# excamera/alfalfa

Hardware: AMD Instinct MI355X
Metric: 1080p macroblocks/s decode (bit-exact vs reference) (higher is better)
Workload: dtype u8

## Files before the change

### alfalfa_amd/csrc/kernels.hip

```cpp
#include <hip/hip_runtime.h>
#include <algorithm>
#include <cstddef>

#include <cstdlib>

#include "device_types.h"
#include "vp8_math.hh"
#include "coeff_pack.hh"
#include "recon_inl.hh"

namespace aa {
namespace {
using namespace recon;

constexpr int kLanes = 64;

enum : int { DC_PRED, V_PRED, H_PRED, TM_PRED, B_PRED, NEARESTMV, NEARMV, ZEROMV, NEWMV, SPLITMV };

struct alignas( 16 ) ResidualLds {
  union {
    int16_t cf[25][16];
    int16_t res[24][16];
  };
  int16_t im[24][16];
  uint8_t map[32];
};

__device__ void compute_residual( const aa_mb_info & mb, const aa_dev_frame & f, ResidualLds & L, const int lane )
{
  uint32_t * z = reinterpret_cast<uint32_t *>( &L.cf[0][0] );
  for ( int i = lane; i < 200; i += kLanes ) z[i] = 0;
  const uint32_t mask = mb.nz_mask;
  if ( lane < 25 && ( ( mask >> lane ) & 1u ) ) L.map[lane == 24 ? 0 : __popc( mask & ( ( 1u << lane ) - 1u ) ) + static_cast<int>( mask >> 24 )] = static_cast<uint8_t>( lane );
  __syncthreads();
  const uint16_t * q = f.quant[mb.segment_id & 3];
  if ( f.packed ) {
    const int16_t * const w = f.coeffs + ( static_cast<size_t>( mb.reserved ) << 32 | mb.coeff_index );
    uint16_t * const scr = reinterpret_cast<uint16_t *>( &L.im[0][0] );
    if ( lane < 25 ) scr[lane] = ( ( mask >> lane ) & 1u ) ? static_cast<uint16_t>( w[lane] ) : 0u;
    __syncthreads();
    if ( lane < 25 ) {
      uint32_t off = pack::kMaskSlots;
      if ( lane != 24 ) { off += __popc( scr[24] ); for ( int b = 0; b < lane; b++ ) off += __popc( scr[b] ); }
      scr[32 + lane] = static_cast<uint16_t>( off );
    }
    __syncthreads();
    for ( int k = lane; k < 25 * 16; k += kLanes ) {
      const int blk = k >> 4, e = k & 15;
      const uint32_t m = scr[blk], zz = pack::zigzag_of( e );
      if ( ( m >> zz ) & 1u ) {
        const int base = blk < 16 ? 0 : ( blk < 24 ? 4 : 2 );
        L.cf[blk][e] = static_cast<int16_t>( dequant( w[scr[32 + blk] + __popc( m & ( ( 1u << zz ) - 1u ) )], q[base + ( e ? 1 : 0 )] ) );
      }
    }
  } else {
    const int n = __popc( mask ) * 16;
    const int16_t * src = f.coeffs + static_cast<size_t>( mb.coeff_index ) * 16;
    for ( int k = lane; k < n; k += kLanes ) {
      const int blk = L.map[k >> 4], e = k & 15;
      const int base = blk < 16 ? 0 : ( blk < 24 ? 4 : 2 );
      L.cf[blk][e] = static_cast<int16_t>( dequant( src[k], q[base + ( e ? 1 : 0 )] ) );
    }
  }
  __syncthreads();
  if ( mb.flags & AA_MB_HAS_Y2 ) {
    if ( lane < 4 ) {
      const Quad v = iwht_pass1( L.cf[24][lane], L.cf[24][lane + 4], L.cf[24][lane + 8], L.cf[24][lane + 12] );
      L.im[0][lane] = static_cast<int16_t>( v.v0 ); L.im[0][lane + 4] = static_cast<int16_t>( v.v1 );
      L.im[0][lane + 8] = static_cast<int16_t>( v.v2 ); L.im[0][lane + 12] = static_cast<int16_t>( v.v3 );
    }
    __syncthreads();
    if ( lane < 4 ) {
      const int o = lane * 4;
      const Quad v = iwht_pass2( L.im[0][o], L.im[0][o + 1], L.im[0][o + 2], L.im[0][o + 3] );
      L.cf[o + 0][0] = static_cast<int16_t>( v.v0 ); L.cf[o + 1][0] = static_cast<int16_t>( v.v1 );
      L.cf[o + 2][0] = static_cast<int16_t>( v.v2 ); L.cf[o + 3][0] = static_cast<int16_t>( v.v3 );
    }
    __syncthreads();
  }
  for ( int t = lane; t < 96; t += kLanes ) {
    const int blk = t >> 2, i = t & 3;
    const Quad v = idct_pass1( L.cf[blk][i], L.cf[blk][i + 4], L.cf[blk][i + 8], L.cf[blk][i + 12] );
    L.im[blk][i * 4 + 0] = static_cast<int16_t>( v.v0 ); L.im[blk][i * 4 + 1] = static_cast<int16_t>( v.v1 );
    L.im[blk][i * 4 + 2] = static_cast<int16_t>( v.v2 ); L.im[blk][i * 4 + 3] = static_cast<int16_t>( v.v3 );
  }
  __syncthreads();
  for ( int t = lane; t < 96; t += kLanes ) {
    const int blk = t >> 2, i = t & 3;
    const Quad v = idct_pass2( L.im[blk][i], L.im[blk][i + 4], L.im[blk][i + 8], L.im[blk][i + 12] );
    L.res[blk][i * 4 + 0] = static_cast<int16_t>( v.v0 ); L.res[blk][i * 4 + 1] = static_cast<int16_t>( v.v1 );
    L.res[blk][i * 4 + 2] = static_cast<int16_t>( v.v2 ); L.res[blk][i * 4 + 3] = static_cast<int16_t>( v.v3 );
  }
  __syncthreads();
}

__device__ __forceinline__ int clampi( int v, int lo, int hi ) { return v < lo ? lo : ( v > hi ? hi : v ); }

__device__ __forceinline__ void load_taps( int frac, int ( &t )[6] )
{
  for ( int i = 0; i < 6; i++ ) t[i] = sixtap_coeff( frac, i );
}

__device__ __forceinline__ uint32_t bytes_at( const uint32_t d0, const uint32_t d1, const uint32_t d2, const int s )
{
  const int q = s >> 2, sh = s & 3;
  const uint32_t lo = q == 0 ? d0 : ( q == 1 ? d1 : d2 );
  const uint32_t hi = q == 0 ? d1 : ( q == 1 ? d2 : 0u );
  return __builtin_amdgcn_alignbyte( hi, lo, sh );
}
__device__ __forceinline__ uint32_t sixtap_x4( uint32_t d0, uint32_t d1, uint32_t d2, const int o, const int frac, const uint32_t t0123, const uint32_t t45 )
{
  if ( frac == 0 ) return bytes_at( d0, d1, d2, o + 2 );
  d0 ^= 0x80808080u; d1 ^= 0x80808080u; d2 ^= 0x80808080u;
  uint32_t out = 0;
#pragma unroll
  for ( int k = 0; k < 4; k++ ) {
    const int a = static_cast<int>( bytes_at( d0, d1, d2, o + k ) ), b = static_cast<int>( bytes_at( d0, d1, d2, o + k + 4 ) );
    int v = __builtin_amdgcn_sdot4( a, static_cast<int>( t0123 ), __builtin_amdgcn_sdot4( b, static_cast<int>( t45 ), 16384 + 64, false ), false ) >> 7;
    asm volatile( "" : "+v"( v ) );
    out |= static_cast<uint32_t>( clamp255( v ) ) << ( 8 * k );
  }
  return out;
}

struct alignas( 16 ) InterLds {
  ResidualLds r;
  alignas( 16 ) uint8_t pred[384];
  union {
    struct {
      uint32_t sw[24][9][3];
      uint32_t st[24][4][3];
      int16_t unit[24][6];
    };
    struct {
      uint32_t wy[21][6], wc[2][13][4];
      uint32_t ty[16][6], tc[2][8][4];
    };
  };
};

__device__ __forceinline__ void recon_inter_body( const aa_dev_frame & f, const unsigned bx, const unsigned max_mbs, InterLds & L, const bool split_only )
{
  const unsigned total = static_cast<unsigned>( f.mbw ) * f.mbh;
  const unsigned chunk = ( max_mbs + 7u ) >> 3;
  const unsigned mi = ( bx & 7u ) * chunk + ( bx >> 3 );
  if ( mi >= total ) return;
  const aa_mb_info & mb = f.mbs[mi];
  if ( !( mb.flags & AA_MB_INTER ) ) return;
  if ( split_only && mb.y_mode != SPLITMV ) return;
  const int lane = threadIdx.x;
  const int col = mi % f.mbw, row = mi / f.mbw;
  const int pw = f.mbw * 16, ph = f.mbh * 16, cw = pw >> 1, ch = ph >> 1;
  const bool has_res = mb.flags & AA_MB_HAS_NONZERO;
  const uint8_t * const * ref = f.ref[mb.ref_frame & 3];
  const bool whole = mb.y_mode != SPLITMV;
  const int mvx = mb.u.mv[0][0], mvy = mb.u.mv[0][1];
  const int cmx = chroma_mv( 4 * mvx ), cmy = chroma_mv( 4 * mvy );
// ... 796 lines not shown
      if ( on && !inside ) {
        uint8_t * by = &S.wy[0][0];
        for ( int i = l; i < 21 * 24; i += 16 ) {
          const int r = i / 24, c = i % 24;
          by[i] = ref_y[static_cast<size_t>( clampi( syy + r, 0, ph - 1 ) ) * pw + clampi( sxy + c, 0, pw - 1 )];
        }
        uint8_t * bc = &S.wc[0][0][0];
        for ( int i = l; i < 2 * 13 * 16; i += 16 ) {
          const int pl = i / 208, e = i % 208, r = e >> 4, c = e & 15;
          bc[i] = ( pl ? ref_v : ref_u )[static_cast<size_t>( clampi( syc + r, 0, ch - 1 ) ) * cw + clampi( sxc + c, 0, cw - 1 )];
        }
      }
    }
  }
  const int oy = inside ? ( sxy & 3 ) : 0, oc = inside ? ( sxc & 3 ) : 0;
  __syncthreads();

  const bool luma_general = __any( on && ( ( mvx | mvy ) & 7 ) != 0 ), chroma_general = __any( on && ( ( cmx | cmy ) & 7 ) != 0 );
  const uint8_t * const wyb = &S.wy[0][0]; const uint8_t * const wcb = &S.wc[0][0][0];
  uint8_t * const tyb = &S.ty[0][0]; uint8_t * const tcb = &S.tc[0][0][0];
  if ( on && luma_general ) {
    const int frac = mvx & 7;
    const uint32_t t0 = L.taps[2 * frac], t1 = L.taps[2 * frac + 1];
#pragma unroll
    for ( int k = 0; k < 6; k++ ) {
      const int t = l + 16 * k;
      if ( k == 5 && t >= 84 ) continue;
      const int r = t >> 2, g = t & 3;
      const uint8_t * sp = wyb + r * 24 + g * 4;
      const uint32_t o4 = sixtap_x4_lane( *reinterpret_cast<const uint32_t *>( sp ), *reinterpret_cast<const uint32_t *>( sp + 4 ), *reinterpret_cast<const uint32_t *>( sp + 8 ), oy, frac, t0, t1 );
      uint8_t * tb = tyb + ( g * 4 ) * 24 + r;
      tb[0] = static_cast<uint8_t>( o4 ); tb[24] = static_cast<uint8_t>( o4 >> 8 ); tb[48] = static_cast<uint8_t>( o4 >> 16 ); tb[72] = static_cast<uint8_t>( o4 >> 24 );
    }
  }
  if ( on && chroma_general ) {
    const int frac = cmx & 7;
    const uint32_t t0 = L.taps[2 * frac], t1 = L.taps[2 * frac + 1];
#pragma unroll
    for ( int k = 0; k < 4; k++ ) {
      const int j = l + 16 * k;
      if ( k == 3 && j >= 52 ) continue;
      const int pl = j >= 26 ? 1 : 0, e = j - 26 * pl, r = e >> 1, g = e & 1;
      const uint8_t * sp = wcb + pl * 208 + r * 16 + g * 4;
      const uint32_t o4 = sixtap_x4_lane( *reinterpret_cast<const uint32_t *>( sp ), *reinterpret_cast<const uint32_t *>( sp + 4 ), *reinterpret_cast<const uint32_t *>( sp + 8 ), oc, frac, t0, t1 );
      uint8_t * tb = tcb + pl * 128 + ( g * 4 ) * 16 + r;
      tb[0] = static_cast<uint8_t>( o4 ); tb[16] = static_cast<uint8_t>( o4 >> 8 ); tb[32] = static_cast<uint8_t>( o4 >> 16 ); tb[48] = static_cast<uint8_t>( o4 >> 24 );
    }
  }
  uint4 copy_y = make_uint4( 0, 0, 0, 0 ); uint2 copy_c = make_uint2( 0, 0 );
  if ( !luma_general && on ) {
    const uint2 * rp = reinterpret_cast<const uint2 *>( wyb + ( l + 2 ) * 24 );
    const uint2 a = rp[0], b = rp[1], c = rp[2];
    const bool q = oy + 2 >= 4; const int sft = ( oy + 2 ) & 3;
    const uint32_t e0 = q ? a.y : a.x, e1 = q ? b.x : a.y, e2 = q ? b.y : b.x, e3 = q ? c.x : b.y, e4 = q ? c.y : c.x;
    copy_y = make_uint4( __builtin_amdgcn_alignbyte( e1, e0, sft ), __builtin_amdgcn_alignbyte( e2, e1, sft ),
                         __builtin_amdgcn_alignbyte( e3, e2, sft ), __builtin_amdgcn_alignbyte( e4, e3, sft ) );
  }
  if ( !chroma_general && on ) {
    const int pl = l >> 3, r = l & 7;
    const uint2 * rp = reinterpret_cast<const uint2 *>( wcb + pl * 208 + ( r + 2 ) * 16 );
    const uint2 a = rp[0], b = rp[1];
    const bool q = oc + 2 >= 4; const int sft = ( oc + 2 ) & 3;
    const uint32_t e0 = q ? a.y : a.x, e1 = q ? b.x : a.y, e2 = q ? b.y : b.x;
    copy_c = make_uint2( __builtin_amdgcn_alignbyte( e1, e0, sft ), __builtin_amdgcn_alignbyte( e2, e1, sft ) );
  }
  __syncthreads();
  if ( !luma_general && on ) *reinterpret_cast<uint4 *>( S.pred + l * 16 ) = copy_y;
  if ( !chroma_general && on ) *reinterpret_cast<uint2 *>( S.pred + 256 + ( l >> 3 ) * 64 + ( l & 7 ) * 8 ) = copy_c;
  if ( on && luma_general ) {
    const int frac = mvy & 7;
    const uint32_t t0 = L.taps[2 * frac], t1 = L.taps[2 * frac + 1];
#pragma unroll
    for ( int k = 0; k < 4; k++ ) {
      const int t = l + 16 * k, c = t >> 2, i = t & 3;
      const uint8_t * sp = tyb + c * 24 + i * 4;
      const uint32_t o4 = sixtap_x4_lane( *reinterpret_cast<const uint32_t *>( sp ), *reinterpret_cast<const uint32_t *>( sp + 4 ), *reinterpret_cast<const uint32_t *>( sp + 8 ), 0, frac, t0, t1 );
      uint8_t * pb = S.pred + ( i * 4 ) * 16 + c;
      pb[0] = static_cast<uint8_t>( o4 ); pb[16] = static_cast<uint8_t>( o4 >> 8 ); pb[32] = static_cast<uint8_t>( o4 >> 16 ); pb[48] = static_cast<uint8_t>( o4 >> 24 );
    }
  }
  if ( on && chroma_general ) {
    const int frac = cmy & 7;
    const uint32_t t0 = L.taps[2 * frac], t1 = L.taps[2 * frac + 1];
#pragma unroll
    for ( int k = 0; k < 2; k++ ) {
      const int j = l + 16 * k, pl = j >> 4, c = ( j >> 1 ) & 7, i = j & 1;
      const uint8_t * sp = tcb + pl * 128 + c * 16 + i * 4;
      const uint32_t o4 = sixtap_x4_lane( *reinterpret_cast<const uint32_t *>( sp ), *reinterpret_cast<const uint32_t *>( sp + 4 ), *reinterpret_cast<const uint32_t *>( sp + 8 ), 0, frac, t0, t1 );
      uint8_t * pb = S.pred + 256 + pl * 64 + ( i * 4 ) * 8 + c;
      pb[0] = static_cast<uint8_t>( o4 ); pb[8] = static_cast<uint8_t>( o4 >> 8 ); pb[16] = static_cast<uint8_t>( o4 >> 16 ); pb[24] = static_cast<uint8_t>( o4 >> 24 );
    }
  }
  __syncthreads();

  if ( on ) {
    uint32_t o[4];
#pragma unroll
    for ( int k = 0; k < 4; k++ ) {
      const uint32_t p4 = *reinterpret_cast<const uint32_t *>( S.pred + l * 16 + 4 * k );
      const uint32_t out = has_res ? add_residual_x4( p4, &S.res[( l >> 2 ) * 4 + k][( l & 3 ) * 4] ) : p4;
      o[k] = out;
    }
    *reinterpret_cast<uint4 *>( f.cur[0] + static_cast<size_t>( row * 16 + l ) * pw + col * 16 ) = make_uint4( o[0], o[1], o[2], o[3] );
    const int pl = l >> 3, r = l & 7;
    uint32_t oc2[2];
#pragma unroll
    for ( int k = 0; k < 2; k++ ) {
      const uint32_t p4 = *reinterpret_cast<const uint32_t *>( S.pred + 256 + pl * 64 + r * 8 + 4 * k );
      const uint32_t out = has_res ? add_residual_x4( p4, &S.res[16 + pl * 4 + ( r >> 2 ) * 2 + k][( r & 3 ) * 4] ) : p4;
      oc2[k] = out;
    }
    *reinterpret_cast<uint2 *>( f.cur[1 + pl] + static_cast<size_t>( row * 8 + r ) * cw + col * 8 ) = make_uint2( oc2[0], oc2[1] );
  }
}

__global__ __launch_bounds__( kLanes ) void k_recon_inter4( const aa_frame_list list, const unsigned max_quads )
{
  __builtin_amdgcn_s_setprio( 3 );

  __shared__ Inter4Lds L;
  recon_inter4_body( *list.f[blockIdx.y], blockIdx.x, max_quads, L );
}

constexpr int kStripMbs = 8;
constexpr int kStripRow = 16 + 16 * kStripMbs;
constexpr int kStripRpi = 16 / kStripMbs;
static_assert( ( kStripRow / 16 ) % 2 == 1, "odd multiple of 16: consecutive rows start on different banks" );
struct alignas( 16 ) LfStrip {
  uint8_t c[12][kStripRow];
  uint8_t y[20][kStripRow];
  uint8_t halo_y[16][4];
  uint8_t halo_c[2][8][4];
  uint8_t pad[32];
};
struct alignas( 16 ) LfStripLds { LfStrip slot[4]; };

__device__ __forceinline__ uint64_t load_u64_shared( const uint8_t * p )
{
  return __hip_atomic_load( reinterpret_cast<const uint64_t *>( p ), __ATOMIC_RELAXED, __HIP_MEMORY_SCOPE_AGENT );
}

__device__ __forceinline__ void lf_edges_pk( pk2 ( &v )[20], const LfParamsPk & P, const pk2 g0, const pk2 g1, const pk2 g23 )
{
  if ( __any( g0 != 0u ) ) lf_edge_pk( P, true, g0, v[0], v[1], v[2], v[3], v[4], v[5], v[6], v[7] );
  if ( __any( g1 != 0u ) ) {
    lf_edge_pk( P, false, g1, v[4], v[5], v[6], v[7], v[8], v[9], v[10], v[11] );
    if ( __any( g23 != 0u ) ) {
      lf_edge_pk( P, false, g23, v[8], v[9], v[10], v[11], v[12], v[13], v[14], v[15] );
      lf_edge_pk( P, false, g23, v[12], v[13], v[14], v[15], v[16], v[17], v[18], v[19] );
    }
  }
}

__device__ __forceinline__ void loopfilter_strip_row( const aa_frame_list & list, const int group, const int row, const int mbh_max, const int mbw_max,
                                                       aa_sync_ws * ws, uint8_t * bnd, LfStripLds & S, const int dbg, const int home_xcc )
{
  const int lane = threadIdx.x, slot = lane >> 4, l = lane & 15;
  const aa_dev_frame & f0 = *list.f[group * 4];
  const int mbh = f0.mbh;
  if ( row >= mbh ) return;
  const aa_dev_frame * const fp = list.f[group * 4 + slot];
  const bool frame_on = fp != nullptr && fp->loop_filter_level != 0;
  if ( !__any( frame_on ) ) return;
  const aa_dev_frame & f = fp ? *fp : f0;
  LfStrip & T = S.slot[slot];
  int * const progress = ws->progress + group * mbh_max;
  const int mbw = f0.mbw, pw = mbw * 16, cw = pw >> 1;
  const int y0 = row * 16, cy0 = row * 8;
  const int sharp = f.sharpness; const bool key = f.key_frame;
  const bool last_row = row == mbh - 1;
  const bool luma = l < 8;
  const int k8 = l & 7, cp = k8 >> 2, cj = k8 & 3;
  uint8_t * const vrow = luma ? &T.y[4 + 2 * l][16] : &T.c[4 + 2 * cj][16 + 8 * kStripMbs * cp];
  uint8_t * const vhalo = luma ? &T.halo_y[2 * l][0] : &T.halo_c[cp][2 * cj][0];
  uint8_t * const hcol = luma ? &T.y[0][16 + 2 * l] : &T.c[0][16 + 8 * kStripMbs * cp + 2 * cj];
  const int mbstep = luma ? 16 : 8;
  const int brow = l / kStripMbs, bchunk = l % kStripMbs;
  uint8_t * const gy = f.cur[0] + static_cast<size_t>( y0 + brow ) * pw + 16 * bchunk;
  uint8_t * const gu = f.cur[1] + static_cast<size_t>( cy0 + brow ) * cw + 8 * bchunk;
  uint8_t * const gv = f.cur[2] + static_cast<size_t>( cy0 + brow ) * cw + 8 * bchunk;
  uint8_t * const sy = &T.y[4 + brow][16 + 16 * bchunk];
  uint8_t * const sc = &T.c[4 + brow][16 + 8 * bchunk];
  const int bl = l & 7, bq = ( bl - 4 ) & 3;
  uint8_t * const bsrc = bl < 4 ? &T.y[16 + bl][16] : &T.c[8 + 2 * ( bq & 1 )][16 + 8 * kStripMbs * ( bq >> 1 )];
  uint8_t * const btop = bl < 4 ? &T.y[bl][16] : &T.c[2 * ( bq & 1 )][16 + 8 * kStripMbs * ( bq >> 1 )];
  const int bstep = bl < 4 ? 16 : 8;
  const size_t bnd_row = ( static_cast<size_t>( group * 4 + slot ) * mbh_max + row ) * mbw_max;
  uint8_t * const bnd_own = bnd + bnd_row * 128 + 16 * bl;
  const uint8_t * const bnd_top = bnd + ( bnd_row - mbw_max ) * 128 + 16 * bl;
  const int fq = l >> 2, fr = l & 3;
  const int fix_off = fq == 0 ? 16 * fr + 12 : 64 + 32 * ( fq - 1 ) + 8 * fr + 4;
  uint8_t * const fix_src0 = fq == 0 ? &T.halo_y[12 + fr][0] : &T.halo_c[( fq - 1 ) & 1][4 + fr][0];
  uint8_t * const fix_srck = fq == 0 ? &T.y[16 + fr][16 - 4] : &T.c[8 + fr][16 + 8 * kStripMbs * ( ( fq - 1 ) & 1 ) - 4];
  const int fix_step = fq == 0 ? 16 : 8;
  uint8_t * const fy = f.cur[0] + static_cast<size_t>( y0 + l ) * pw - 4;
  uint8_t * const fc = f.cur[1 + ( l >> 3 )] + static_cast<size_t>( cy0 + ( l & 7 ) ) * cw - 4;
  const aa_mb_info * const mbrow = f.mbs + static_cast<size_t>( row ) * mbw;

  const int n_strips = ( mbw + kStripMbs - 1 ) / kStripMbs;
  uint4 py[kStripMbs]; uint2 pc[kStripMbs];
#pragma unroll
  for ( int i = 0; i < kStripMbs; i++ ) { py[i] = make_uint4( 0, 0, 0, 0 ); pc[i] = make_uint2( 0, 0 ); }
  auto prefetch = [&]( const int s ) {
    const bool in = frame_on && !( dbg & 2 ) && s * kStripMbs + bchunk < mbw;
    if ( in ) {
#pragma unroll
      for ( int i = 0; i < kStripMbs; i++ ) py[i] = *reinterpret_cast<const uint4 *>( gy + static_cast<size_t>( kStripRpi * i ) * pw + 16 * kStripMbs * s );
#pragma unroll
      for ( int i = 0; i < kStripMbs / 2; i++ ) pc[i] = *reinterpret_cast<const uint2 *>( gu + static_cast<size_t>( kStripRpi * i ) * cw + 8 * kStripMbs * s );
#pragma unroll
      for ( int i = 0; i < kStripMbs / 2; i++ ) pc[kStripMbs / 2 + i] = *reinterpret_cast<const uint2 *>( gv + static_cast<size_t>( kStripRpi * i ) * cw + 8 * kStripMbs * s );
    }
  };
  prefetch( 0 );
  int info = frame_on ? *reinterpret_cast<const uint16_t *>( &mbrow[0].flags ) : 0;
  int seen = row > 0 ? 0 : mbw;
  LfParamsPk P = lf_params_pk( lf_params( 1, sharp, key ) );
  int p_level = -1;
  for ( int s = 0; s < n_strips; s++ ) {
    const int nmb = min( kStripMbs, mbw - s * kStripMbs );
    if ( s > 0 ) {
      *reinterpret_cast<uint32_t *>( &T.halo_y[l][0] ) = *reinterpret_cast<const uint32_t *>( &T.y[4 + l][16 + 16 * kStripMbs - 4] );
      *reinterpret_cast<uint32_t *>( &T.halo_c[l >> 3][l & 7][0] ) = *reinterpret_cast<const uint32_t *>( &T.c[4 + ( l & 7 )][16 + 8 * kStripMbs * ( l >> 3 ) + 8 * kStripMbs - 4] );
      __syncthreads();
    }
#pragma unroll
    for ( int i = 0; i < kStripMbs; i++ ) *reinterpret_cast<uint4 *>( sy + kStripRpi * kStripRow * i ) = py[i];
#pragma unroll
    for ( int i = 0; i < kStripMbs / 2; i++ ) { *reinterpret_cast<uint2 *>( sc + kStripRpi * kStripRow * i ) = pc[i]; *reinterpret_cast<uint2 *>( sc + kStripRpi * kStripRow * i + 8 * kStripMbs ) = pc[kStripMbs / 2 + i]; }
    __syncthreads();

    for ( int k = 0; k < nmb; k++ ) {
      const int col = s * kStripMbs + k;
      const int level = info >> 8;
      const bool active = level != 0;
      const bool inner = !( info & AA_MB_LF_SKIP_INNER );
      const bool more = col + 1 < mbw;
      const int info_next = ( frame_on && more ) ? *reinterpret_cast<const uint16_t *>( &mbrow[col + 1].flags ) : 0;
      const int need = col + 1;
      if ( row > 0 && seen < need ) seen = poll_progress( &progress[row - 1] );
      const bool any_active = __any( active );
      if ( !__all( level == p_level ) ) { P = lf_params_pk( lf_params( active ? level : 1, sharp, key ) ); p_level = level; }
      const pk2 g_on = active ? ~0u : 0u, g_in = ( active && inner ) ? ~0u : 0u, g_in23 = ( active && inner && luma ) ? ~0u : 0u;

      if ( any_active && !( dbg & 4 ) ) {
        uint8_t * const ra = vrow + mbstep * k;
        uint8_t * const ha = k == 0 ? vhalo : ra - 4;
        uint8_t * const hb = k == 0 ? vhalo + 4 : ra + kStripRow - 4;
        uint32_t a[5], b[5];
        a[0] = *reinterpret_cast<const uint32_t *>( ha ); b[0] = *reinterpret_cast<const uint32_t *>( hb );
        { const uint2 u = *reinterpret_cast<const uint2 *>( ra ); a[1] = u.x; a[2] = u.y; }
        { const uint2 u = *reinterpret_cast<const uint2 *>( ra + 8 ); a[3] = u.x; a[4] = u.y; }
        { const uint2 u = *reinterpret_cast<const uint2 *>( ra + kStripRow ); b[1] = u.x; b[2] = u.y; }
        { const uint2 u = *reinterpret_cast<const uint2 *>( ra + kStripRow + 8 ); b[3] = u.x; b[4] = u.y; }
        pk2 v[20];
#pragma unroll
        for ( int d = 0; d < 5; d++ ) {
          v[4 * d] = pk_from_bytes<0>( a[d], b[d] ); v[4 * d + 1] = pk_from_bytes<1>( a[d], b[d] );
          v[4 * d + 2] = pk_from_bytes<2>( a[d], b[d] ); v[4 * d + 3] = pk_from_bytes<3>( a[d], b[d] );
        }
        lf_edges_pk( v, P, col > 0 ? g_on : 0u, g_in, g_in23 );
#pragma unroll
        for ( int d = 0; d < 5; d++ ) pk_to_dwords( v[4 * d], v[4 * d + 1], v[4 * d + 2], v[4 * d + 3], a[d], b[d] );
        if ( active ) {
          *reinterpret_cast<uint32_t *>( ha ) = a[0]; *reinterpret_cast<uint32_t *>( hb ) = b[0];
          *reinterpret_cast<uint2 *>( ra ) = make_uint2( a[1], a[2] ); *reinterpret_cast<uint2 *>( ra + kStripRow ) = make_uint2( b[1], b[2] );
          if ( luma ) { *reinterpret_cast<uint2 *>( ra + 8 ) = make_uint2( a[3], a[4] ); *reinterpret_cast<uint2 *>( ra + kStripRow + 8 ) = make_uint2( b[3], b[4] ); }
        }
      }
      __syncthreads();
      if ( frame_on && !last_row && col > 0 && l < 12 && !( dbg & 1 ) ) {
        const uint8_t * src = k == 0 ? fix_src0 : fix_srck + fix_step * k;
        *reinterpret_cast<uint32_t *>( bnd + ( bnd_row + col - 1 ) * 128 + fix_off ) = *reinterpret_cast<const uint32_t *>( src );
      }

      if ( row > 0 ) {
        if ( !( dbg & 16 ) ) wait_for_row_above( true, need, seen, 2, ws, progress, group, row, mbh, home_xcc, lf_min_polls( dbg ), lf_max_wait_ticks( dbg ) );

        if ( frame_on && l < 8 && !( dbg & 8 ) ) {
          const uint8_t * src = bnd_top + static_cast<size_t>( col ) * 128;
          const uint64_t lo = load_u64_shared( src ), hi = load_u64_shared( src + 8 );
          uint8_t * dst = btop + bstep * k;
          if ( bl < 4 ) { *reinterpret_cast<uint64_t *>( dst ) = lo; *reinterpret_cast<uint64_t *>( dst + 8 ) = hi; }
          else { *reinterpret_cast<uint64_t *>( dst ) = lo; *reinterpret_cast<uint64_t *>( dst + kStripRow ) = hi; }
        }
      }
      publish_progress( lane == 0 && col > 0 && !lf_fault_injected( dbg, row ), &progress[row], col );
      if ( k == 0 && s + 1 < n_strips ) prefetch( s + 1 );
      __syncthreads();

      if ( any_active && !( dbg & 4 ) ) {
        uint8_t * const hc = hcol + mbstep * k;
        pk2 v[20];
#pragma unroll
        for ( int r = 0; r < 20; r++ ) v[r] = pk_from_u16( *reinterpret_cast<const uint16_t *>( hc + kStripRow * r ) );
        lf_edges_pk( v, P, row > 0 ? g_on : 0u, g_in, g_in23 );
        if ( active ) {
#pragma unroll
          for ( int r = 1; r < 12; r++ ) *reinterpret_cast<uint16_t *>( hc + kStripRow * r ) = static_cast<uint16_t>( pk_to_u16( v[r] ) );
          if ( luma ) {
#pragma unroll
            for ( int r = 12; r < 20; r++ ) *reinterpret_cast<uint16_t *>( hc + kStripRow * r ) = static_cast<uint16_t>( pk_to_u16( v[r] ) );
          }
        }
      }
      __syncthreads();

      if ( frame_on && !( dbg & 1 ) ) {
        if ( !last_row ) {
          if ( l < 8 ) {
            const uint8_t * src = bsrc + bstep * k;
            uint4 q;
            if ( bl < 4 ) q = *reinterpret_cast<const uint4 *>( src );
            else { const uint2 u0 = *reinterpret_cast<const uint2 *>( src ), u1 = *reinterpret_cast<const uint2 *>( src + kStripRow ); q = make_uint4( u0.x, u0.y, u1.x, u1.y ); }
            *reinterpret_cast<uint4 *>( bnd_own + static_cast<size_t>( col ) * 128 ) = q;
          }
        }
        if ( k == 0 && s > 0 ) {
          if ( l < 12 || last_row ) *reinterpret_cast<uint32_t *>( fy + 16 * kStripMbs * s ) = *reinterpret_cast<const uint32_t *>( &T.halo_y[l][0] );
          if ( ( l & 7 ) < 4 || last_row ) *reinterpret_cast<uint32_t *>( fc + 8 * kStripMbs * s ) = *reinterpret_cast<const uint32_t *>( &T.halo_c[l >> 3][l & 7][0] );
        }
        if ( k == nmb - 1 && bchunk < nmb ) {
#pragma unroll
          for ( int i = 0; i < 20 / kStripRpi; i++ ) {
            if ( ( ( i + 1 ) * kStripRpi > 4 || row > 0 ) && ( i * kStripRpi < 16 || last_row ) )
              *reinterpret_cast<uint4 *>( gy + ( static_cast<ptrdiff_t>( kStripRpi * i ) - 4 ) * pw + 16 * kStripMbs * s ) = *reinterpret_cast<const uint4 *>( sy + kStripRpi * kStripRow * i - 4 * kStripRow );
          }
#pragma unroll
          for ( int i = 0; i < 12 / kStripRpi; i++ ) {
            if ( ( ( i + 1 ) * kStripRpi > 4 || row > 0 ) && ( i * kStripRpi < 8 || last_row ) ) {
              *reinterpret_cast<uint2 *>( gu + ( static_cast<ptrdiff_t>( kStripRpi * i ) - 4 ) * cw + 8 * kStripMbs * s ) = *reinterpret_cast<const uint2 *>( sc + kStripRpi * kStripRow * i - 4 * kStripRow );
              *reinterpret_cast<uint2 *>( gv + ( static_cast<ptrdiff_t>( kStripRpi * i ) - 4 ) * cw + 8 * kStripMbs * s ) = *reinterpret_cast<const uint2 *>( sc + kStripRpi * kStripRow * i - 4 * kStripRow + 8 * kStripMbs );
            }
          }
        }
      }
      info = info_next;
      __syncthreads();
    }
  }
  publish_progress( lane == 0 && !lf_fault_injected( dbg, row ), &progress[row], mbw );
}

__device__ __forceinline__ void loopfilter_rows4_body( const aa_frame_list & list, const int n_groups, const int mbh_max, const int mbw_max, aa_sync_ws * ws, uint8_t * bnd,
                                                        const int n_xcd, LfStripLds & S, int & s_ticket, const int dbg )
{
  const int xcc = xcc_id();
  if ( xcc >= n_xcd ) { if ( threadIdx.x == 0 ) atomicExch( &ws->error, 3 ); return; }
  for ( ;; ) {
    const int t = take_ticket( ws, xcc, &s_ticket, threadIdx.x );
    const int mine = xcc < n_groups ? ( n_groups - xcc + n_xcd - 1 ) / n_xcd : 0;
    if ( t >= mine * mbh_max ) return;
    loopfilter_strip_row( list, ( t % mine ) * n_xcd + xcc, t / mine, mbh_max, mbw_max, ws, bnd, S, dbg, xcc );
  }
}

__global__ __launch_bounds__( kLanes ) __attribute__( ( amdgpu_waves_per_eu( 2 ) ) ) void k_loopfilter_rows4( const aa_frame_list list, const int n_groups, const int mbh_max, const int mbw_max, aa_sync_ws * ws, uint8_t * bnd,
                                                                 const int n_xcd, const int dbg )
{
  __builtin_amdgcn_s_setprio( 3 );

  __shared__ LfStripLds S;
  __shared__ int s_ticket;
  loopfilter_rows4_body( list, n_groups, mbh_max, mbw_max, ws, bnd, n_xcd, S, s_ticket, dbg );
}

__global__ void k_probe_xcds( int * out )
{
  if ( threadIdx.x == 0 ) atomicAdd( &out[xcc_id() & 15], 1 );
}

__global__ void k_probe_concurrency( uint32_t * counter, uint32_t * seen, uint32_t n, unsigned long long timeout, int slot )
{
  if ( threadIdx.x || blockIdx.x ) return;
  __hip_atomic_fetch_add( counter, 1u, __ATOMIC_RELAXED, __HIP_MEMORY_SCOPE_AGENT );
  const unsigned long long t0 = wall_clock64();
  uint32_t m;
  while ( ( m = __hip_atomic_load( counter, __ATOMIC_RELAXED, __HIP_MEMORY_SCOPE_AGENT ) ) < n && wall_clock64() - t0 < timeout ) __builtin_amdgcn_s_sleep( 32 );
  seen[slot] = m;
}

__global__ void k_check_tickets( aa_sync_ws * ws, const int n_groups, const int mbh_max, const int n_xcd )
{
  if ( threadIdx.x != 0 || blockIdx.x != 0 ) return;
  for ( int x = 0; x < n_xcd; x++ ) {
    const int mine = x < n_groups ? ( n_groups - x + n_xcd - 1 ) / n_xcd : 0;
    const int t = __hip_atomic_load( &ws->ticket[x], __ATOMIC_RELAXED, __HIP_MEMORY_SCOPE_AGENT );
    if ( t < mine * mbh_max && atomicCAS( &ws->error, 0, 5 ) == 0 ) { ws->where[0] = x; ws->where[1] = t; ws->where[2] = mine * mbh_max; }
  }
}

__global__ void k_bind_rasters( const aa_raster_binding * b, int n )
{
  const int i = blockIdx.x * blockDim.x + threadIdx.x;
  if ( i >= n ) return;
  aa_dev_frame * f = b[i].job;
  for ( int p = 0; p < 3; p++ ) f->cur[p] = b[i].cur[p];
  for ( int r = 1; r < 4; r++ ) for ( int p = 0; p < 3; p++ ) f->ref[r][p] = b[i].ref[r - 1][p];
}

__global__ __launch_bounds__( 256 ) void k_gather_rasters( const aa_gather_job * jobs, uint8_t * staging, size_t stride )
{
  const aa_gather_job J = jobs[blockIdx.y];
  const uint4 * src = reinterpret_cast<const uint4 *>( J.src );
  uint4 * dst = reinterpret_cast<uint4 *>( staging + stride * blockIdx.y );
  const size_t n16 = J.bytes >> 4;
  for ( size_t i = size_t( blockIdx.x ) * 256 + threadIdx.x; i < n16; i += size_t( gridDim.x ) * 256 ) dst[i] = src[i];
  if ( blockIdx.x == 0 && threadIdx.x < ( J.bytes & 15 ) ) staging[stride * blockIdx.y + ( n16 << 4 ) + threadIdx.x] = J.src[( n16 << 4 ) + threadIdx.x];
}

constexpr int kRgbCy = 76309, kRgbCrv = 104574, kRgbCgu = 25642, kRgbCgv = 53281, kRgbCbu = 132213;

template <int ESZ, int N>
__device__ inline void rgb_store( uint8_t * p, const uint32_t ( &e )[N], const int n, const bool fast )
{
  static_assert( ( N * ESZ ) % 16 == 0, "whole 16-byte pieces" );
  if ( fast ) {
    uint32_t w[N * ESZ / 4];
#pragma unroll
    for ( int i = 0; i < N * ESZ / 4; i++ ) {
      if ( ESZ == 1 ) w[i] = e[4 * i] | e[4 * i + 1] << 8 | e[4 * i + 2] << 16 | e[4 * i + 3] << 24;
      else if ( ESZ == 2 ) w[i] = ( e[2 * i] & 0xFFFFu ) | e[2 * i + 1] << 16;
      else w[i] = e[i];
    }
    uint4 * q = reinterpret_cast<uint4 *>( p );
#pragma unroll
    for ( int i = 0; i < N * ESZ / 16; i++ ) q[i] = make_uint4( w[4 * i], w[4 * i + 1], w[4 * i + 2], w[4 * i + 3] );
    return;
  }
#pragma unroll
  for ( int i = 0; i < N; i++ )
    if ( i < n )
#pragma unroll
      for ( int b = 0; b < ESZ; b++ ) p[i * ESZ + b] = static_cast<uint8_t>( e[i] >> ( 8 * b ) );
}

template <int F>
__global__ __launch_bounds__( 256 ) void k_render_rgb( const aa_rgb_job * jobs, const uint32_t * table )
{
  constexpr bool kFloat = F >= AA_RGB_F16_CHW;
  constexpr int kEsz = F == AA_RGB_F32_CHW ? 4 : F >= AA_RGB_F16_CHW ? 2 : 1;
  __shared__ uint32_t T[kFloat ? 768 : 1];
  if ( kFloat ) {
    for ( int i = threadIdx.x; i < 768; i += 256 ) T[i] = table[i];
    __syncthreads();
  }
  const aa_rgb_job & J = jobs[blockIdx.y];
  const uint32_t groups = J.groups, w = J.width, h = J.height;
  const uint32_t t = blockIdx.x * 256u + threadIdx.x;
  if ( t >= groups * ( ( h + 1 ) >> 1 ) ) return;
  const int k = static_cast<int>( t / groups ), x0 = static_cast<int>( t - uint32_t( k ) * groups ) * 16;
  const int cw = static_cast<int>( ( w + 1 ) >> 1 ), ch = static_cast<int>( ( h + 1 ) >> 1 );
  const int j0 = x0 >> 1, je = min( j0 + 8, cw - 1 );
  const int crow[3] = { max( k - 1, 0 ), k, min( k + 1, ch - 1 ) };
  int c[2][3][9];
#pragma unroll
  for ( int p = 0; p < 2; p++ )
#pragma unroll
    for ( int r = 0; r < 3; r++ ) {
      const uint8_t * row = J.plane[1 + p] + size_t( crow[r] ) * J.stride_c;
      const uint2 q = *reinterpret_cast<const uint2 *>( row + j0 );
      c[p][r][8] = row[je];
#pragma unroll
      for ( int i = 0; i < 8; i++ ) {
        const int b = static_cast<int>( ( ( i < 4 ? q.x : q.y ) >> ( 8 * ( i & 3 ) ) ) & 255u );
        c[p][r][i] = j0 + i > je ? c[p][r][8] : b;
      }
    }
  const int n = min( 16, static_cast<int>( w ) - x0 );
  for ( int r = 0; r < 2; r++ ) {
    const int y = 2 * k + r;
    if ( y >= static_cast<int>( h ) ) continue;
    const uint4 yq = *reinterpret_cast<const uint4 *>( J.plane[0] + size_t( y ) * J.stride_y + x0 );
    const uint32_t yw[4] = { yq.x, yq.y, yq.z, yq.w };
    int v[2][9];
#pragma unroll
    for ( int p = 0; p < 2; p++ )
#pragma unroll
      for ( int i = 0; i < 9; i++ ) v[p][i] = 3 * c[p][1][i] + c[p][r ? 2 : 0][i];
    uint32_t R[16], G[16], B[16];
#pragma unroll
    for ( int i = 0; i < 16; i++ ) {
      const int Y = static_cast<int>( ( yw[i >> 2] >> ( 8 * ( i & 3 ) ) ) & 255u );
      const int j = i >> 1;
      const int u8 = ( i & 1 ) ? v[0][j] + v[0][j + 1] : 2 * v[0][j];
      const int v8 = ( i & 1 ) ? v[1][j] + v[1][j + 1] : 2 * v[1][j];
      const int yt = 8 * kRgbCy * ( Y - 16 ), ut = u8 - 1024, vt = v8 - 1024;
      R[i] = static_cast<uint32_t>( min( max( ( yt + kRgbCrv * vt + ( 1 << 18 ) ) >> 19, 0 ), 255 ) );
      G[i] = static_cast<uint32_t>( min( max( ( yt - kRgbCgu * ut - kRgbCgv * vt + ( 1 << 18 ) ) >> 19, 0 ), 255 ) );
      B[i] = static_cast<uint32_t>( min( max( ( yt + kRgbCbu * ut + ( 1 << 18 ) ) >> 19, 0 ), 255 ) );
    }
    uint8_t * const row = J.dst + y * J.row_stride;
    if ( F == AA_RGB_U8_HWC3 || F == AA_RGB_U8_HWC4 ) {
      constexpr int C = F == AA_RGB_U8_HWC3 ? 3 : 4;
      uint32_t e[16 * C];
#pragma unroll
      for ( int i = 0; i < 16; i++ ) {
        e[C * i] = R[i]; e[C * i + 1] = G[i]; e[C * i + 2] = B[i];
        if ( C == 4 ) e[C * i + 3] = 255u;
      }
      uint8_t * const p = row + x0 * C;
      rgb_store<1, 16 * C>( p, e, n * C, n == 16 && !( reinterpret_cast<uintptr_t>( p ) & 15 ) );
    } else {
#pragma unroll
      for ( int ci = 0; ci < 3; ci++ ) {
        const uint32_t * const src = ci == 0 ? R : ci == 1 ? G : B;
        uint32_t e[16];
#pragma unroll
        for ( int i = 0; i < 16; i++ ) e[i] = kFloat ? T[ci * 256 + src[i]] : src[i];
        uint8_t * const p = row + ci * J.plane_stride + x0 * kEsz;
        rgb_store<kEsz, 16>( p, e, n, n == 16 && !( reinterpret_cast<uintptr_t>( p ) & 15 ) );
      }
    }
  }
}

}

__global__ __launch_bounds__( 256 ) void k_lf_relevel( const aa_mb_info * src, aa_mb_info * dst, unsigned nmb, uint32_t levels )
{
  const unsigned i = blockIdx.x * blockDim.x + threadIdx.x;
  if ( i >= nmb ) return;
  const uint4 * s = reinterpret_cast<const uint4 *>( src + i );
  uint4 * d = reinterpret_cast<uint4 *>( dst + i );
  uint4 head = s[0];
  const uint32_t seg = ( head.x >> 24 ) & 3u;
  head.y = ( head.y & 0xFFFF00FFu ) | ( ( ( levels >> ( 8 * seg ) ) & 255u ) << 8 );
  d[0] = head;
  for ( int k = 1; k < 5; k++ ) d[k] = s[k];
}
static_assert( sizeof( aa_mb_info ) == 80, "k_lf_relevel copies five 16-byte pieces" );

int launch_lf_relevel( const aa_mb_info * src, aa_mb_info * dst, unsigned nmb, uint32_t levels, void * stream )
{
  hipLaunchKernelGGL( k_lf_relevel, dim3( ( nmb + 255 ) / 256 ), dim3( 256 ), 0, static_cast<hipStream_t>( stream ), src, dst, nmb, levels );
  return static_cast<int>( hipGetLastError() );
}

int launch_gather_rasters( const aa_gather_job * jobs, int n, uint8_t * staging, size_t stride, size_t max_bytes, void * stream )
{
  const unsigned per = static_cast<unsigned>( std::min<size_t>( 64, std::max<size_t>( 1, max_bytes / ( 256 * 16 * 4 ) ) ) );
  for ( int base = 0; base < n; base += 32768 ) {
    const int cnt = std::min( 32768, n - base );
    hipLaunchKernelGGL( k_gather_rasters, dim3( per, cnt ), dim3( 256 ), 0, static_cast<hipStream_t>( stream ), jobs + base, staging + stride * base, stride );
    if ( hipError_t e = hipGetLastError() ) return static_cast<int>( e );
  }
  return 0;
}

int launch_render_rgb( const aa_rgb_job * jobs, int n, int format, const uint32_t * table, uint32_t max_threads, void * stream )
{
  const unsigned blocks = ( max_threads + 255u ) / 256u;
  const hipStream_t st = static_cast<hipStream_t>( stream );
  for ( int base = 0; base < n; base += 32768 ) {
    const dim3 grid( blocks, std::min( 32768, n - base ) );
    switch ( format ) {
      case AA_RGB_U8_HWC3: hipLaunchKernelGGL( k_render_rgb<AA_RGB_U8_HWC3>, grid, dim3( 256 ), 0, st, jobs + base, table ); break;
      case AA_RGB_U8_HWC4: hipLaunchKernelGGL( k_render_rgb<AA_RGB_U8_HWC4>, grid, dim3( 256 ), 0, st, jobs + base, table ); break;
      case AA_RGB_U8_CHW: hipLaunchKernelGGL( k_render_rgb<AA_RGB_U8_CHW>, grid, dim3( 256 ), 0, st, jobs + base, table ); break;
      case AA_RGB_F16_CHW: hipLaunchKernelGGL( k_render_rgb<AA_RGB_F16_CHW>, grid, dim3( 256 ), 0, st, jobs + base, table ); break;
      case AA_RGB_BF16_CHW: hipLaunchKernelGGL( k_render_rgb<AA_RGB_BF16_CHW>, grid, dim3( 256 ), 0, st, jobs + base, table ); break;
      case AA_RGB_F32_CHW: hipLaunchKernelGGL( k_render_rgb<AA_RGB_F32_CHW>, grid, dim3( 256 ), 0, st, jobs + base, table ); break;
      default: return static_cast<int>( hipErrorInvalidValue );
    }
    if ( hipError_t e = hipGetLastError() ) return static_cast<int>( e );
  }
  return 0;
}

int launch_bind_rasters( const aa_raster_binding * b, int n, void * stream )
{
  hipLaunchKernelGGL( k_bind_rasters, dim3( ( n + 63 ) / 64 ), dim3( 64 ), 0, static_cast<hipStream_t>( stream ), b, n );
  return static_cast<int>( hipGetLastError() );
}

int launch_recon_inter( const aa_frame_list & list, int n, unsigned max_mbs, bool split_only, void * stream )
{
  const unsigned blocks = ( ( max_mbs + 7u ) >> 3 ) * 8u;
  hipLaunchKernelGGL( k_recon_inter, dim3( blocks, n ), dim3( kLanes ), 0, static_cast<hipStream_t>( stream ), list, max_mbs, split_only ? 1 : 0 );
  return static_cast<int>( hipGetLastError() );
}
int launch_recon_inter4( const aa_frame_list & list, int n, unsigned max_mbs, void * stream )
{
  const unsigned quads = ( max_mbs + 3u ) >> 2;
  const unsigned blocks = ( ( quads + 7u ) >> 3 ) * 8u;
  hipLaunchKernelGGL( k_recon_inter4, dim3( blocks, n ), dim3( kLanes ), 0, static_cast<hipStream_t>( stream ), list, quads );
  return static_cast<int>( hipGetLastError() );
}
int launch_recon_intra_diagonal( const aa_frame_list & list, int n, int diagonal, int row_lo, int rows, void * stream )
{
  hipLaunchKernelGGL( k_recon_intra, dim3( rows, n ), dim3( kLanes ), 0, static_cast<hipStream_t>( stream ), list, diagonal, row_lo );
  return static_cast<int>( hipGetLastError() );
}
int launch_loopfilter_diagonal( const aa_frame_list & list, int n, int diagonal, int row_lo, int rows, void * stream )
{
  hipLaunchKernelGGL( k_loopfilter, dim3( rows, n ), dim3( kLanes ), 0, static_cast<hipStream_t>( stream ), list, diagonal, row_lo );
  return static_cast<int>( hipGetLastError() );
}
static int lf_debug_bits()
{
  static const int bits = [] { const char * e = std::getenv( "ALFALFA_AMD_LF_DEBUG" ); return e ? std::atoi( e ) : 0; }();
  return bits;
}
static unsigned test_lds_pad()
{
  static const unsigned pad = [] { const char * e = std::getenv( "ALFALFA_AMD_TEST_LDS_PAD" ); return e ? static_cast<unsigned>( std::atoi( e ) ) : 0u; }();
  return pad;
}
int launch_loopfilter_rows4( const aa_frame_list & list, int n_groups, int mbh_max, int mbw_max, aa_sync_ws * ws, uint8_t * boundary, int n_xcd, void * stream )
{
  hipLaunchKernelGGL( k_loopfilter_rows4, dim3( n_xcd * ( ( n_groups + n_xcd - 1 ) / n_xcd ) * mbh_max ), dim3( kLanes ), test_lds_pad(), static_cast<hipStream_t>( stream ), list, n_groups, mbh_max, mbw_max, ws, boundary, n_xcd, lf_debug_bits() );
  hipLaunchKernelGGL( k_check_tickets, dim3( 1 ), dim3( 64 ), 0, static_cast<hipStream_t>( stream ), ws, n_groups, mbh_max, n_xcd );
  return static_cast<int>( hipGetLastError() );
}
int launch_recon_intra4( const aa_frame_list & list, int n_groups, int mbh_max, aa_sync_ws * ws, int n_xcd, void * stream )
{
  hipLaunchKernelGGL( k_recon_intra4, dim3( n_xcd * ( ( n_groups + n_xcd - 1 ) / n_xcd ) * mbh_max ), dim3( kLanes ), test_lds_pad(), static_cast<hipStream_t>( stream ), list, n_groups, mbh_max, ws, n_xcd );
  hipLaunchKernelGGL( k_check_tickets, dim3( 1 ), dim3( 64 ), 0, static_cast<hipStream_t>( stream ), ws, n_groups, mbh_max, n_xcd );
  return static_cast<int>( hipGetLastError() );
}
int launch_probe_concurrency( uint32_t * counter, uint32_t * seen, uint32_t n, unsigned long long timeout_ticks, int slot, void * stream )
{
  hipLaunchKernelGGL( k_probe_concurrency, dim3( 1 ), dim3( 64 ), 0, static_cast<hipStream_t>( stream ), counter, seen, n, timeout_ticks, slot );
  return static_cast<int>( hipGetLastError() );
}
int launch_probe_xcds( int * out16, int blocks, void * stream )
{
  hipLaunchKernelGGL( k_probe_xcds, dim3( blocks ), dim3( kLanes ), 0, static_cast<hipStream_t>( stream ), out16 );
  return static_cast<int>( hipGetLastError() );
}

}
```

Baseline: 123.5 million.

## Add strip-granular progress handoff variant for row loop filter with heuristic selection

```diff
diff --git a/alfalfa_amd/csrc/kernels.hip b/alfalfa_amd/csrc/kernels.hip
--- a/alfalfa_amd/csrc/kernels.hip
+++ b/alfalfa_amd/csrc/kernels.hip
@@ -3,6 +3,7 @@
 #include <cstddef>
 
 #include <cstdlib>
+#include <cstring>
 
 #include "device_types.h"
 #include "vp8_math.hh"
@@ -1105,6 +1106,7 @@
   }
 }
 
+template <bool kStripHandoff>
 __device__ __forceinline__ void loopfilter_strip_row( const aa_frame_list & list, const int group, const int row, const int mbh_max, const int mbw_max,
                                                        aa_sync_ws * ws, uint8_t * bnd, LfStripLds & S, const int dbg, const int home_xcc )
 {
@@ -1166,10 +1168,186 @@
     }
   };
   prefetch( 0 );
-  int info = frame_on ? *reinterpret_cast<const uint16_t *>( &mbrow[0].flags ) : 0;
   int seen = row > 0 ? 0 : mbw;
   LfParamsPk P = lf_params_pk( lf_params( 1, sharp, key ) );
   int p_level = -1;
+  if constexpr ( kStripHandoff ) {
+  auto opaque = []( int v ) { asm volatile( "" : "+v"( v ) ); return v; };
+  auto line_fixup = [&]( const int c0 ) {
+    const int o = opaque( l ), q = o >> 2, r = o & 3;
+    if ( o >= 12 ) return;
+    const int off = ( q == 0 ? 16 * r + 12 : 64 + 32 * ( q - 1 ) + 8 * r + 4 ) - 16 * ( o & 7 );
+    const uint8_t * src = q == 0 ? &T.halo_y[12 + r][0] : &T.halo_c[( q - 1 ) & 1][4 + r][0];
+    *reinterpret_cast<uint32_t *>( bnd_own + static_cast<ptrdiff_t>( c0 - 1 ) * 128 + off ) = *reinterpret_cast<const uint32_t *>( src );
+  };
+  const ptrdiff_t bnd_up = -static_cast<ptrdiff_t>( mbw_max ) * 128;
+  struct MbGates { bool active, any_active; pk2 g_on, g_in, g_in23; };
+  auto begin_mb = [&]( const int info ) {
+    const int level = info >> 8;
+    const bool inner = !( info & AA_MB_LF_SKIP_INNER ), active = level != 0;
+    if ( !__all( level == p_level ) ) { P = lf_params_pk( lf_params( active ? level : 1, sharp, key ) ); p_level = level; }
+    return MbGates{ active, __any( active ) != 0, active ? ~0u : 0u, ( active && inner ) ? ~0u : 0u, ( active && inner && luma ) ? ~0u : 0u };
+  };
+  auto v_phase = [&]( const int k, const int col, const MbGates & G ) {
+    if ( !G.any_active || ( dbg & 4 ) ) return;
+    uint8_t * const ra = vrow + mbstep * k;
+    uint8_t * const ha = k == 0 ? vhalo : ra - 4;
+    uint8_t * const hb = k == 0 ? vhalo + 4 : ra + kStripRow - 4;
+    uint32_t a[5], b[5];
+    a[0] = *reinterpret_cast<const uint32_t *>( ha ); b[0] = *reinterpret_cast<const uint32_t *>( hb );
+    { const uint2 u = *reinterpret_cast<const uint2 *>( ra ); a[1] = u.x; a[2] = u.y; }
+    { const uint2 u = *reinterpret_cast<const uint2 *>( ra + 8 ); a[3] = u.x; a[4] = u.y; }
+    { const uint2 u = *reinterpret_cast<const uint2 *>( ra + kStripRow ); b[1] = u.x; b[2] = u.y; }
+    { const uint2 u = *reinterpret_cast<const uint2 *>( ra + kStripRow + 8 ); b[3] = u.x; b[4] = u.y; }
+    pk2 v[20];
+#pragma unroll
+    for ( int d = 0; d < 5; d++ ) {
+      v[4 * d] = pk_from_bytes<0>( a[d], b[d] ); v[4 * d + 1] = pk_from_bytes<1>( a[d], b[d] );
+      v[4 * d + 2] = pk_from_bytes<2>( a[d], b[d] ); v[4 * d + 3] = pk_from_bytes<3>( a[d], b[d] );
+    }
+    lf_edges_pk( v, P, col > 0 ? G.g_on : 0u, G.g_in, G.g_in23 );
+#pragma unroll
+    for ( int d = 0; d < 5; d++ ) pk_to_dwords( v[4 * d], v[4 * d + 1], v[4 * d + 2], v[4 * d + 3], a[d], b[d] );
+    if ( G.active ) {
+      *reinterpret_cast<uint32_t *>( ha ) = a[0]; *reinterpret_cast<uint32_t *>( hb ) = b[0];
+      *reinterpret_cast<uint2 *>( ra ) = make_uint2( a[1], a[2] ); *reinterpret_cast<uint2 *>( ra + kStripRow ) = make_uint2( b[1], b[2] );
+      if ( luma ) { *reinterpret_cast<uint2 *>( ra + 8 ) = make_uint2( a[3], a[4] ); *reinterpret_cast<uint2 *>( ra + kStripRow + 8 ) = make_uint2( b[3], b[4] ); }
+    }
+  };
+  auto h_phase = [&]( const int k, const MbGates & G ) {
+    if ( !G.any_active || ( dbg & 4 ) ) return;
+    uint8_t * const hc = hcol + mbstep * k;
+    pk2 v[20];
+#pragma unroll
+    for ( int r = 0; r < 20; r++ ) v[r] = pk_from_u16( *reinterpret_cast<const uint16_t *>( hc + kStripRow * r ) );
+    lf_edges_pk( v, P, row > 0 ? G.g_on : 0u, G.g_in, G.g_in23 );
+    if ( G.active ) {
+#pragma unroll
+      for ( int r = 1; r < 12; r++ ) *reinterpret_cast<uint16_t *>( hc + kStripRow * r ) = static_cast<uint16_t>( pk_to_u16( v[r] ) );
+      if ( luma ) {
+#pragma unroll
+        for ( int r = 12; r < 20; r++ ) *reinterpret_cast<uint16_t *>( hc + kStripRow * r ) = static_cast<uint16_t>( pk_to_u16( v[r] ) );
+      }
+    }
+  };
+  auto frame_fixup = [&]( const int s ) {
+    const int o = opaque( l ), ob = o / kStripMbs, oc = o % kStripMbs;
+    uint8_t * const fy = gy + static_cast<ptrdiff_t>( o - ob ) * pw - 16 * oc - 4 + 16 * kStripMbs * s;
+    uint8_t * const fc = ( o >> 3 ? gv : gu ) + static_cast<ptrdiff_t>( ( o & 7 ) - ob ) * cw - 8 * oc - 4 + 8 * kStripMbs * s;
+    if ( o < 12 || last_row ) *reinterpret_cast<uint32_t *>( fy ) = *reinterpret_cast<const uint32_t *>( &T.halo_y[o][0] );
+    if ( ( o & 7 ) < 4 || last_row ) *reinterpret_cast<uint32_t *>( fc ) = *reinterpret_cast<const uint32_t *>( &T.halo_c[o >> 3][o & 7][0] );
+  };
+  auto store_strip = [&]( const int s ) {
+#pragma unroll
+    for ( int i = 0; i < 20 / kStripRpi; i++ ) {
+      if ( ( ( i + 1 ) * kStripRpi > 4 || row > 0 ) && ( i * kStripRpi < 16 || last_row ) )
+        *reinterpret_cast<uint4 *>( gy + ( static_cast<ptrdiff_t>( kStripRpi * i ) - 4 ) * pw + 16 * kStripMbs * s ) = *reinterpret_cast<const uint4 *>( sy + kStripRpi * kStripRow * i - 4 * kStripRow );
+    }
+#pragma unroll
+    for ( int i = 0; i < 12 / kStripRpi; i++ ) {
+      if ( ( ( i + 1 ) * kStripRpi > 4 || row > 0 ) && ( i * kStripRpi < 8 || last_row ) ) {
+        *reinterpret_cast<uint2 *>( gu + ( static_cast<ptrdiff_t>( kStripRpi * i ) - 4 ) * cw + 8 * kStripMbs * s ) = *reinterpret_cast<const uint2 *>( sc + kStripRpi * kStripRow * i - 4 * kStripRow );
+        *reinterpret_cast<uint2 *>( gv + ( static_cast<ptrdiff_t>( kStripRpi * i ) - 4 ) * cw + 8 * kStripMbs * s ) = *reinterpret_cast<const uint2 *>( sc + kStripRpi * kStripRow * i - 4 * kStripRow + 8 * kStripMbs );
+      }
+    }
+  };
+  auto turn_over = [&]( const int s ) {
+    if ( s > 0 ) {
+      *reinterpret_cast<uint32_t *>( &T.halo_y[l][0] ) = *reinterpret_cast<const uint32_t *>( &T.y[4 + l][16 + 16 * kStripMbs - 4] );
+      *reinterpret_cast<uint32_t *>( &T.halo_c[l >> 3][l & 7][0] ) = *reinterpret_cast<const uint32_t *>( &T.c[4 + ( l & 7 )][16 + 8 * kStripMbs * ( l >> 3 ) + 8 * kStripMbs - 4] );
+      __syncthreads();
+    }
+#pragma unroll
+    for ( int i = 0; i < kStripMbs; i++ ) *reinterpret_cast<uint4 *>( sy + kStripRpi * kStripRow * i ) = py[i];
+#pragma unroll
+    for ( int i = 0; i < kStripMbs / 2; i++ ) { *reinterpret_cast<uint2 *>( sc + kStripRpi * kStripRow * i ) = pc[i]; *reinterpret_cast<uint2 *>( sc + kStripRpi * kStripRow * i + 8 * kStripMbs ) = pc[kStripMbs / 2 + i]; }
+  };
+
+  static_assert( kStripMbs == 8, "two 128-byte boundary lines per instruction of 16 lanes, four instructions per strip" );
+  const int tm = l >> 3;
+  uint64_t tq[kStripMbs];
+#pragma unroll
+  for ( int i = 0; i < kStripMbs; i++ ) tq[i] = 0;
+  auto load_top = [&]( const int s ) {
+#pragma unroll
+    for ( int i = 0; i < kStripMbs / 2; i++ ) {
+      const int c = s * kStripMbs + 2 * i + tm;
+      if ( frame_on && !( dbg & 8 ) && c < mbw ) {
+        const uint8_t * src = bnd_own + bnd_up + static_cast<size_t>( c ) * 128;
+        tq[2 * i] = load_u64_shared( src ); tq[2 * i + 1] = load_u64_shared( src + 8 );
+      }
+    }
+  };
+  auto drop_top = [&]() {
+#pragma unroll
+    for ( int i = 0; i < kStripMbs / 2; i++ ) {
+      uint8_t * dst = btop + bstep * ( 2 * i + tm );
+      *reinterpret_cast<uint64_t *>( dst ) = tq[2 * i];
+      *reinterpret_cast<uint64_t *>( dst + ( bl < 4 ? 8 : kStripRow ) ) = tq[2 * i + 1];
+    }
+  };
+  auto load_infos = [&]( const int s ) {
+    const int c = s * kStripMbs + l;
+    return ( frame_on && l < kStripMbs && c < mbw ) ? static_cast<int>( *reinterpret_cast<const uint16_t *>( &mbrow[c].flags ) ) : 0;
+  };
+  int infos_next = load_infos( 0 );
+  bool top_ahead = false;
+  for ( int s = 0; s < n_strips; s++ ) {
+    const int c0 = s * kStripMbs, nmb = min( kStripMbs, mbw - c0 );
+    const int need = c0 + nmb;
+    if ( row > 0 && seen < need ) seen = poll_progress( &progress[row - 1] );
+    turn_over( s );
+    if ( top_ahead ) drop_top();
+    const int infos = infos_next;
+    __syncthreads();
+
+    for ( int k = 0; k < nmb; k++ ) {
+      const MbGates G = begin_mb( __shfl( infos, k, 16 ) );
+      v_phase( k, c0 + k, G );
+      __syncthreads();
+      if ( k == 0 ) {
+        if ( s > 0 ) {
+          if ( frame_on && !( dbg & 1 ) ) {
+            if ( !last_row ) line_fixup( c0 );
+            frame_fixup( s );
+          }
+          publish_progress( lane == 0 && !lf_fault_injected( dbg, row ), &progress[row], c0 );
+        }
+        if ( row > 0 && !( dbg & 16 ) ) wait_for_row_above( true, need, seen, 2, ws, progress, group, row, mbh, home_xcc, lf_min_polls( dbg ), lf_max_wait_ticks( dbg ) );
+        if ( row > 0 && !top_ahead ) { load_top( s ); drop_top(); }
+        top_ahead = false;
+        if ( s + 1 < n_strips ) {
+          prefetch( s + 1 );
+          infos_next = load_infos( s + 1 );
+          top_ahead = row > 0 && __all( seen >= min( c0 + 2 * kStripMbs, mbw ) );
+          if ( top_ahead ) load_top( s + 1 );
+        }
+        __syncthreads();
+      }
+      h_phase( k, G );
+      __syncthreads();
+    }
+
+    if ( frame_on && !( dbg & 1 ) ) {
+      if ( bchunk < nmb ) store_strip( s );
+      if ( !last_row ) {
+#pragma unroll
+        for ( int i = 0; i < kStripMbs / 2; i++ ) {
+          const int m = 2 * i + tm;
+          if ( m < nmb ) {
+            const uint8_t * src = bsrc + bstep * m;
+            uint4 q;
+            if ( bl < 4 ) q = *reinterpret_cast<const uint4 *>( src );
+            else { const uint2 u0 = *reinterpret_cast<const uint2 *>( src ), u1 = *reinterpret_cast<const uint2 *>( src + kStripRow ); q = make_uint4( u0.x, u0.y, u1.x, u1.y ); }
+            *reinterpret_cast<uint4 *>( bnd_own + static_cast<size_t>( c0 + m ) * 128 ) = q;
+          }
+        }
+      }
+    }
+    __syncthreads();
+  }
+  } else {
+  int info = frame_on ? *reinterpret_cast<const uint16_t *>( &mbrow[0].flags ) : 0;
   for ( int s = 0; s < n_strips; s++ ) {
     const int nmb = min( kStripMbs, mbw - s * kStripMbs );
     if ( s > 0 ) {
@@ -1292,9 +1470,11 @@
       __syncthreads();
     }
   }
+  }
   publish_progress( lane == 0 && !lf_fault_injected( dbg, row ), &progress[row], mbw );
 }
 
+template <bool kStripHandoff>
 __device__ __forceinline__ void loopfilter_rows4_body( const aa_frame_list & list, const int n_groups, const int mbh_max, const int mbw_max, aa_sync_ws * ws, uint8_t * bnd,
                                                         const int n_xcd, LfStripLds & S, int & s_ticket, const int dbg )
 {
@@ -1304,10 +1484,11 @@
     const int t = take_ticket( ws, xcc, &s_ticket, threadIdx.x );
     const int mine = xcc < n_groups ? ( n_groups - xcc + n_xcd - 1 ) / n_xcd : 0;
     if ( t >= mine * mbh_max ) return;
-    loopfilter_strip_row( list, ( t % mine ) * n_xcd + xcc, t / mine, mbh_max, mbw_max, ws, bnd, S, dbg, xcc );
-  }
-}
-
+    loopfilter_strip_row<kStripHandoff>( list, ( t % mine ) * n_xcd + xcc, t / mine, mbh_max, mbw_max, ws, bnd, S, dbg, xcc );
+  }
+}
+
+template <bool kStripHandoff>
 __global__ __launch_bounds__( kLanes ) __attribute__( ( amdgpu_waves_per_eu( 2 ) ) ) void k_loopfilter_rows4( const aa_frame_list list, const int n_groups, const int mbh_max, const int mbw_max, aa_sync_ws * ws, uint8_t * bnd,
                                                                  const int n_xcd, const int dbg )
 {
@@ -1315,7 +1496,7 @@
 
   __shared__ LfStripLds S;
   __shared__ int s_ticket;
-  loopfilter_rows4_body( list, n_groups, mbh_max, mbw_max, ws, bnd, n_xcd, S, s_ticket, dbg );
+  loopfilter_rows4_body<kStripHandoff>( list, n_groups, mbh_max, mbw_max, ws, bnd, n_xcd, S, s_ticket, dbg );
 }
 
 __global__ void k_probe_xcds( int * out )
@@ -1560,9 +1741,22 @@
   static const unsigned pad = [] { const char * e = std::getenv( "ALFALFA_AMD_TEST_LDS_PAD" ); return e ? static_cast<unsigned>( std::atoi( e ) ) : 0u; }();
   return pad;
 }
+static bool lf_strip_handoff( const int n_groups, const int mbh_max, const int mbw_max, const int n_xcd )
+{
+  static const int forced = [] { const char * e = std::getenv( "ALFALFA_AMD_LF_HANDOFF" ); return !e ? 0 : !std::strcmp( e, "strip" ) ? 1 : !std::strcmp( e, "mb" ) ? 2 : 0; }();
+  if ( forced ) return forced == 1;
+  static const int cus = [] { int dev = 0, n = 0; if ( hipGetDevice( &dev ) != hipSuccess || hipDeviceGetAttribute( &n, hipDeviceAttributeMultiprocessorCount, dev ) != hipSuccess ) n = 0; return n; }();
+  const long long resident = 3ll * max( 1, cus / max( 1, n_xcd ) );
+  const long long rows = static_cast<long long>( ( n_groups + n_xcd - 1 ) / n_xcd ) * mbh_max;
+  return rows * mbw_max >= resident * ( mbw_max + ( kStripMbs + 1ll ) * ( mbh_max - 1 ) );
+}
 int launch_loopfilter_rows4( const aa_frame_list & list, int n_groups, int mbh_max, int mbw_max, aa_sync_ws * ws, uint8_t * boundary, int n_xcd, void * stream )
 {
-  hipLaunchKernelGGL( k_loopfilter_rows4, dim3( n_xcd * ( ( n_groups + n_xcd - 1 ) / n_xcd ) * mbh_max ), dim3( kLanes ), test_lds_pad(), static_cast<hipStream_t>( stream ), list, n_groups, mbh_max, mbw_max, ws, boundary, n_xcd, lf_debug_bits() );
+  const dim3 grid( n_xcd * ( ( n_groups + n_xcd - 1 ) / n_xcd ) * mbh_max );
+  if ( lf_strip_handoff( n_groups, mbh_max, mbw_max, n_xcd ) )
+    hipLaunchKernelGGL( k_loopfilter_rows4<true>, grid, dim3( kLanes ), test_lds_pad(), static_cast<hipStream_t>( stream ), list, n_groups, mbh_max, mbw_max, ws, boundary, n_xcd, lf_debug_bits() );
+  else
+    hipLaunchKernelGGL( k_loopfilter_rows4<false>, grid, dim3( kLanes ), test_lds_pad(), static_cast<hipStream_t>( stream ), list, n_groups, mbh_max, mbw_max, ws, boundary, n_xcd, lf_debug_bits() );
   hipLaunchKernelGGL( k_check_tickets, dim3( 1 ), dim3( 64 ), 0, static_cast<hipStream_t>( stream ), ws, n_groups, mbh_max, n_xcd );
   return static_cast<int>( hipGetLastError() );
 }
```

After: 125.8 million, median of 6. +1.9%, better.
